# ArtOfBBQ/debigulator

Measured on NVIDIA B200. Metric: inflate_output_GBps, higher is better.
Workload: dtype u8

## Files before the change

debigulator_b200/csrc/bsplit_kernels.cuh:

```cuda
#pragma once
#include <cuda_runtime.h>
#include <stdint.h>

#include "bsplit_core.h"
#include "split_kernels.cuh"

namespace dbg {

constexpr uint64_t BS_MIN_BYTES = 65536;
constexpr int BS_WARPS_PER_CTA = 4;

struct BsSummary {
    uint32_t n_split;
    uint32_t total_regions;
    uint64_t total_in;
    uint64_t cells_used;
    uint32_t n_fallback;
    uint32_t pad;
    uint64_t split_in;
    uint64_t tok_bytes;
    uint32_t n_pruned;
    uint32_t pad2;
};

// ... 62 lines not shown
    if (thr < b.min_bytes) thr = b.min_bytes;
    if (b.dyn_all && size >= b.min_bytes && ((b.pre_status && b.pre_status[s]) ? 0u : ((b.in_base[b.in_off[s]] >> 1) & 3)) == 2) thr = b.min_bytes;
    uint32_t flag = 0;
    const bool ok = (!b.pre_status || b.pre_status[s] == 0) && (!b.taken || b.taken[s] == 0) && size >= thr && cap >= size &&
                    size < (1ull << 31) && cap < (1ull << 32) - 1024;
    b.redo[s] = 0;
    const uint32_t first = ok ? b.in_base[b.in_off[s]] : 0u;
    if (ok && ((first >> 1) & 3) != 0 && (first & 1) == 0) {
        flag = 1;
        atomicAdd(&b.summary->n_split, 1u);
        atomicAdd((unsigned long long *)&b.summary->split_in, (unsigned long long)size);
    }
    b.flag[s] = flag;
}

__global__ void bs_assign_kernel(BsBatch b)
{
    const uint32_t s = blockIdx.x * blockDim.x + threadIdx.x;
    if (s >= b.n || !b.flag[s]) return;
    const uint32_t nreg = (uint32_t)((b.in_size[s] + b.region_bytes - 1) / b.region_bytes);
    b.chunk_base[s] = atomicAdd(&b.summary->total_regions, nreg);
    b.nchunks[s] = nreg;
    if (b.tok)
        b.tok_stream_base[s] = (uint64_t)b.tok_per_byte *
                               atomicAdd((unsigned long long *)&b.summary->tok_bytes, (unsigned long long)b.in_size[s]);
}

__global__ void bs_fill_kernel(BsBatch b)
{
    const uint32_t s = blockIdx.x;
    if (!b.flag[s]) return;
    const uint32_t nch = b.nchunks[s], base = b.chunk_base[s];
    for (uint32_t c = threadIdx.x; c < nch; c += blockDim.x) b.chunk_stream[base + c] = s;
}

__global__ void __launch_bounds__(BS_WARPS_PER_CTA * 32) bs_search_kernel(BsBatch b)
{
    const uint32_t total_regions = b.summary->total_regions;
    __shared__ uint16_t kraft12[4096];
    __shared__ SearchSmem qs[BS_WARPS_PER_CTA];
    build_kraft12(kraft12, threadIdx.x, blockDim.x);
    __syncthreads();
    SearchSmem *q = &qs[threadIdx.x >> 5];
    const uint32_t warps = gridDim.x * BS_WARPS_PER_CTA;
    for (uint32_t t = blockIdx.x * BS_WARPS_PER_CTA + (threadIdx.x >> 5); t < total_regions; t += warps) {
        const uint32_t s = b.chunk_stream[t], c = t - b.chunk_base[s];
        uint64_t cand = 0;
        if (c) cand = find_block_start(q, kraft12, b.in_base + b.in_off[s], b.in_size[s], (uint64_t)c * b.region_bytes * 8,
                                       (uint64_t)(c + 1) * b.region_bytes * 8);
        if (simt::lane() == 0) b.cand[t] = cand;
        simt::syncwarp();
    }
}

__global__ void bs_prune_kernel(BsBatch b)
{
    const uint32_t s = blockIdx.x * blockDim.x + threadIdx.x;
    if (s >= b.n || !b.flag[s]) return;
    const uint32_t nch = b.nchunks[s], base = b.chunk_base[s];
    const uint64_t bits = 8 * b.in_size[s];
    uint64_t prev = 0, worst = 0;
    for (uint32_t c = 1; c < nch; c++) {
        const uint64_t cand = b.cand[base + c];
        if (cand == BS_NONE) continue;
        if (cand - prev > worst) worst = cand - prev;
        prev = cand;
    }
    if (bits - prev > worst) worst = bits - prev;
    if (worst > bits / 3) {
        for (uint32_t c = 0; c < nch; c++) b.cand[base + c] = BS_NONE;
        b.redo[s] = 1;
        atomicAdd(&b.summary->n_pruned, 1u);
    }
}

__device__ __forceinline__ uint64_t bs_next_hint(const BsBatch &b, uint32_t s, uint32_t t)
{
    const uint32_t end = b.chunk_base[s] + b.nchunks[s];
    for (uint32_t u = t + 1; u < end; u++)
        if (b.cand[u] != BS_NONE) return b.cand[u];
    return BS_NONE;
}

__global__ void __launch_bounds__(BS_WARPS_PER_CTA * 32) bs_count_kernel(BsBatch b)
{
    const uint32_t total_regions = b.summary->total_regions;
    extern __shared__ __align__(16) uint8_t smem_raw[];
    InflateSmem *sm = reinterpret_cast<InflateSmem *>(smem_raw) + (threadIdx.x >> 5);
    const uint32_t warps = gridDim.x * BS_WARPS_PER_CTA;
    for (uint32_t t = blockIdx.x * BS_WARPS_PER_CTA + (threadIdx.x >> 5); t < total_regions; t += warps) {
        const uint64_t start = b.cand[t];
        if (start == BS_NONE) continue;
        const uint32_t s = b.chunk_stream[t];
        const uint64_t next = bs_next_hint(b, s, t);
        ChunkResult r;
        if (b.tok)
            r = decode_block_chunk<SINK_TOKENS>(sm, b.in_base + b.in_off[s], b.in_size[s], start, next, nullptr, 0, 0,
                                                b.tok + bs_tok_base(b, s, start), bs_tok_cap(b, s, start, next), b.lanes != 0,
                                                b.lb_stats);
        else
            r = decode_block_chunk<SINK_COUNT>(sm, b.in_base + b.in_off[s], b.in_size[s], start, next, nullptr, 0, 0);
        if (simt::lane() == 0) {
            b.exit_bits[t] = r.exit_bits;
            b.c_out_len[t] = r.out_bytes;
            b.c_flag[t] = r.flag;
            if (b.tok) b.c_ntok[t] = r.ntok;
        }
        simt::syncwarp();
    }
}

__global__ void bs_chain_kernel(BsBatch b)
{
    const uint32_t s = blockIdx.x * blockDim.x + threadIdx.x;
    if (s >= b.n || !b.flag[s] || b.redo[s]) return;
    const uint32_t nch = b.nchunks[s], base = b.chunk_base[s];
    const uint64_t cap = b.out_cap[s];
    uint64_t pos = 0, expected = 0;
    uint32_t st = ST_OK;
    bool ended = false, fail = false;
    for (uint32_t c = 0; c < nch; c++) {
        const uint32_t t = base + c;
        const uint64_t cand = b.cand[t];
        const uint32_t len = b.c_out_len[t], flag = b.c_flag[t];
        b.c_out_off[t] = pos;
        if (cand == BS_NONE || ended || fail) {
            b.c_flag[t] = CH_IDLE;
            b.c_out_len[t] = 0;
            continue;
        }
        if (cand < expected) {
            b.c_flag[t] = CH_IDLE;
            b.c_out_len[t] = 0;
            continue;
        }
        if (cand != expected) {
            fail = true;
            b.c_flag[t] = CH_IDLE;
            b.c_out_len[t] = 0;
            continue;
        }
        if (flag >= CH_ERR) {
            st = pos + len > cap ? (uint32_t)ST_OUT_OVERFLOW : flag - CH_ERR;
            ended = true;
            b.c_flag[t] = CH_IDLE;
            b.c_out_len[t] = 0;
            continue;
        }
        pos += len;
        if (pos > cap) {
            st = ST_OUT_OVERFLOW;
            ended = true;
        } else if (flag != CH_RUN) {
            ended = true;
        } else {
            expected = b.exit_bits[t];
        }
    }
    if (!ended) fail = true;
    if (fail) {
        for (uint32_t c = 0; c < nch; c++) {
            b.c_flag[base + c] = CH_IDLE;
            b.c_out_len[base + c] = 0;
        }
        b.redo[s] = 1;
        b.cell_base[s] = 0;
        atomicAdd(&b.summary->n_fallback, 1u);
// ... 134 lines not shown
```

debigulator_b200/csrc/dbg_api.cu:

```cuda
#include <cuda_runtime.h>
#include <stdarg.h>
#include <stdint.h>
#include <stdio.h>
#include <stdlib.h>
#include <string.h>

#include <algorithm>
#include <atomic>
#include <condition_variable>
#include <deque>
#include <mutex>
#include <numeric>
#include <thread>
#include <utility>
#include <vector>

#include "../../include/debigulator_b200.h"
#include "bmp_kernels.cuh"
#include "bsplit_kernels.cuh"
#include "fx_kernels.cuh"
#include "kernels.cuh"
#include "png_kernels.cuh"
#include "split_kernels.cuh"
#include "sprite_kernels.cuh"
// ... 192 lines not shown
    if (const char *v = getenv("DBG_FX_CHUNK")) ctx->fx_chunk_forced = (uint32_t)std::min(1 << 20, std::max((int)dbg::FX_MIN_CHUNK, atoi(v))) & ~15u;
    if (const char *v = getenv("DBG_FX_GROUP")) ctx->fx_group_forced = (uint32_t)std::min(1 << 22, std::max(4096, atoi(v))) & ~15u;
    if (const char *v = getenv("DBG_FX")) ctx->fx = atoi(v) != 0;
    if (const char *v = getenv("DBG_FX_EXPAND_CTAS")) ctx->fx_expand_ctas = (uint32_t)std::min(16, std::max(1, atoi(v)));
    if (const char *v = getenv("DBG_WAVES")) ctx->waves = std::min((int)dbg_ctx::MAX_WAVES, std::max(1, atoi(v)));
    if (const char *v = getenv("DBG_PNG_WAVES")) ctx->png_waves = std::min((int)dbg_ctx::MAX_WAVES, std::max(1, atoi(v)));
    if (const char *v = getenv("DBG_BSPLIT")) ctx->bsplit = atoi(v) != 0;
    if (const char *v = getenv("DBG_BSPLIT_LANES")) ctx->bsplit_lanes = atoi(v) != 0;
    if (const char *v = getenv("DBG_BS_PIECES")) ctx->bs_pieces = atoi(v) != 0;
    if (const char *v = getenv("DBG_ROUNDS")) ctx->rounds = atoi(v) != 0;
    if (const char *v = getenv("DBG_ROUND_BITS")) ctx->round_bits = (uint32_t)std::min(1 << 20, std::max(8192, atoi(v)));
    if (const char *v = getenv("DBG_BSPLIT_ALL")) ctx->bsplit_all = atoi(v);
    if (const char *v = getenv("DBG_BSPLIT_FACTOR_Q")) ctx->bsplit_factor_q = (uint32_t)std::max(1, atoi(v));
    if (const char *v = getenv("DBG_BSPLIT_TOKENS")) ctx->bsplit_tok_per_byte = (uint32_t)std::min(8, std::max(0, atoi(v)));
    if (const char *v = getenv("DBG_BSPLIT_REGION")) ctx->bsplit_region = (uint32_t)std::min(1 << 20, std::max(4096, atoi(v)));
    if (const char *v = getenv("DBG_BSPLIT_REGION_MIN")) ctx->bsplit_region_min = (uint32_t)std::min((int)ctx->bsplit_region, std::max(4096, atoi(v)));
    if (const char *v = getenv("DBG_BSPLIT_MIN_BYTES")) ctx->bsplit_min_bytes = std::max<uint64_t>(strtoull(v, nullptr, 10), 2 * (uint64_t)ctx->bsplit_region);
    if (const char *v = getenv("DBG_INFLATE_CTAS_PER_SM")) {
        int k = atoi(v);
        if (k >= 1 && k <= dbg::INFLATE_CTAS_PER_SM) ctx->inflate_ctas_per_sm = (uint32_t)k;
    }
    return ctx;
}

extern "C" dbg_ctx *dbg_create(int device) { return ctx_create(device, nullptr, 0, nullptr); }

extern "C" void dbg_destroy(dbg_ctx *ctx)
{
    if (!ctx) return;
    cudaSetDevice(ctx->device);
    cudaDeviceSynchronize();
    Buf *all[] = {&ctx->d_in, &ctx->d_out, &ctx->d_desc, &ctx->h_in, &ctx->h_out, &ctx->h_desc, &ctx->d_stats};
    for (Buf *b : all) b->release();
    for (int i = 0; i < dbg_ctx::MAX_WAVES; i++) {
        ctx->slot[i].release();
        Slot &sl = ctx->slot[i];
        if (sl.stream) cudaStreamDestroy(sl.stream);
        if (sl.done) cudaEventDestroy(sl.done);
        if (sl.uploaded) cudaEventDestroy(sl.uploaded);
        if (sl.aux_stream) cudaStreamDestroy(sl.aux_stream);
        if (sl.aux_fork) cudaEventDestroy(sl.aux_fork);
        if (sl.aux_join) cudaEventDestroy(sl.aux_join);
    }
    for (auto &pe : ctx->prof_events) {
        cudaEventDestroy(pe.first);
        cudaEventDestroy(pe.second);
    }
    if (ctx->wave_ready) cudaEventDestroy(ctx->wave_ready);
    if (ctx->up_stream) cudaStreamDestroy(ctx->up_stream);
    if (ctx->stream) cudaStreamDestroy(ctx->stream);
    delete ctx;
}

extern "C" int dbg_bsplit_stats(const dbg_ctx *ctx, uint64_t *streams, uint64_t *fallbacks)
{
    if (!ctx) return DBG_ERR_NO_DEVICE;
    if (streams) *streams = ctx->bs_streams;
    if (fallbacks) *fallbacks = ctx->bs_fallbacks;
    return DBG_OK;
}

extern "C" int dbg_fx_stats(const dbg_ctx *ctx, uint64_t *streams, uint64_t *handed_back, uint64_t *extra_runs)
{
    if (!ctx) return DBG_ERR_NO_DEVICE;
    uint64_t v[3] = {0, 0, 0};
    if (cudaSetDevice(ctx->device) != cudaSuccess || cudaDeviceSynchronize() != cudaSuccess ||
        cudaMemcpy(v, ctx->d_stats.p, sizeof(v), cudaMemcpyDeviceToHost) != cudaSuccess)
        return DBG_ERR_CUDA;
    if (streams) *streams = v[0];
    if (handed_back) *handed_back = v[1];
    if (extra_runs) *extra_runs = v[2];
    return DBG_OK;
}

extern "C" int dbg_lane_stats(const dbg_ctx *ctx, uint32_t v[8])
{
    if (!ctx || !v) return DBG_ERR_ARG;
    if (cudaSetDevice(ctx->device) != cudaSuccess || cudaDeviceSynchronize() != cudaSuccess ||
        cudaMemcpy(v, (uint64_t *)ctx->d_stats.p + 4, 5 * sizeof(uint32_t), cudaMemcpyDeviceToHost) != cudaSuccess ||
        cudaMemcpy(v + 5, (uint64_t *)ctx->d_stats.p + 8, 3 * sizeof(uint32_t), cudaMemcpyDeviceToHost) != cudaSuccess)
        return DBG_ERR_CUDA;
    return DBG_OK;
}

extern "C" int dbg_set_verify(dbg_ctx *ctx, int on)
{
    if (!ctx) return DBG_ERR_ARG;
    ctx->verify = on != 0;
    return DBG_OK;
}

extern "C" int dbg_trim(dbg_ctx *ctx)
{
    if (!ctx) return DBG_ERR_ARG;
    CU(cudaSetDevice(ctx->device));
    CU(cudaDeviceSynchronize());
    for (int i = 0; i < dbg_ctx::MAX_WAVES; i++) ctx->slot[i].release();
    Buf *all[] = {&ctx->d_in, &ctx->d_out, &ctx->d_desc, &ctx->h_in, &ctx->h_out, &ctx->h_desc};
    for (Buf *b : all) b->release();
    return DBG_OK;
}

extern "C" int dbg_profile_enable(dbg_ctx *ctx, int on)
{
    if (!ctx) return DBG_ERR_ARG;
    ctx->profiling = on != 0;
    ctx->prof_used = 0;
    return DBG_OK;
}

extern "C" int dbg_profile_read_tag(dbg_ctx *ctx, int tag, double *total_ms, uint64_t *launches)
{
    if (!ctx || !total_ms || !launches) return DBG_ERR_ARG;
    CU(cudaSetDevice(ctx->device));
    double sum = 0;
    uint64_t cnt = 0;
    for (size_t i = 0; i < ctx->prof_used; i++) {
        if (ctx->prof_tag[i] != tag) continue;
        float ms = 0;
        CU(cudaEventSynchronize(ctx->prof_events[i].second));
        CU(cudaEventElapsedTime(&ms, ctx->prof_events[i].first, ctx->prof_events[i].second));
        sum += ms;
        cnt++;
    }
    *total_ms = sum;
    *launches = cnt;
    return DBG_OK;
}

extern "C" int dbg_profile_read(dbg_ctx *ctx, double *total_ms, uint64_t *launches)
{
    int rc = dbg_profile_read_tag(ctx, DBG_PROF_INFLATE, total_ms, launches);
    if (rc == DBG_OK) ctx->prof_used = 0;
    return rc;
}

extern "C" int dbg_synchronize(dbg_ctx *ctx)
{
    if (!ctx) return DBG_ERR_ARG;
    CU(cudaSetDevice(ctx->device));
    CU(cudaStreamSynchronize(ctx->stream));
    return DBG_OK;
}

struct ProfScope {
    dbg_ctx *ctx;
    cudaStream_t s;
    cudaEvent_t e1 = nullptr;
    ProfScope(dbg_ctx *c, cudaStream_t st, int tag) : ctx(c), s(st)
    {
        if (!ctx->profiling) return;
        std::lock_guard<std::mutex> lock(ctx->prof_mu);
        if (ctx->prof_used == ctx->prof_events.size()) {
            cudaEvent_t a = nullptr, b = nullptr;
            if (cudaEventCreate(&a) != cudaSuccess || cudaEventCreate(&b) != cudaSuccess) return;
            ctx->prof_events.push_back({a, b});
            ctx->prof_tag.push_back(0);
        }
        ctx->prof_tag[ctx->prof_used] = tag;
        cudaEventRecord(ctx->prof_events[ctx->prof_used].first, s);
        e1 = ctx->prof_events[ctx->prof_used].second;
        ctx->prof_used++;
    }
    ~ProfScope()
    {
        if (e1) cudaEventRecord(e1, s);
// ... 1489 lines not shown
```

debigulator_b200/csrc/inflate_core.h:

```cpp
#pragma once
#include "simt.h"

namespace dbg {

enum InflateStatus : uint32_t {
    ST_OK = 0,
    ST_CAP_LT_INPUT = 1,
    ST_INPUT_TOO_SMALL = 2,
    ST_TOO_LARGE = 3,
    ST_STORED_LEN = 4,
    ST_BAD_TABLE = 5,
    ST_BAD_CODE = 6,
    ST_BAD_SYMBOL = 7,
    ST_BAD_DISTANCE = 8,
    ST_OUT_OVERFLOW = 9,
    ST_TRUNCATED = 10,
    ST_BAD_REPEAT = 11,
    ST_CONTAINER = 12,
};

struct InflateSmem {
    uint32_t ring[256];
    uint32_t lit_lut[512];
    uint32_t dist_lut[256];
    uint16_t lit_sorted[288];
    uint16_t lit_first[16], lit_offs[16], lit_cnt[16];
    uint16_t dist_first[16], dist_offs[16], dist_cnt[16];
    uint8_t dist_sorted[32];
    uint8_t lens[320];
    uint32_t cand[2][64];
};

enum { E_LIT = 0x10, E_EOB = 0x20, E_BASE = 0x40, E_BAD = 0x80 };
enum { K_CLEN = 0, K_LITLEN = 1, K_DIST = 2 };
enum { LIT_ROOT = 9, DIST_ROOT = 8 };

template <int KIND>
DBG_DEV uint32_t make_entry(uint32_t sym, uint32_t l)
{
    if (KIND == K_CLEN) return (sym << 16) | E_LIT | l;
    if (KIND == K_LITLEN) {
        if (sym < 256) return (sym << 16) | E_LIT | l;
        if (sym == 256) return E_EOB | l;
        if (sym > 285) return E_BAD | l;
        uint32_t i = sym - 257, xb, base;
        if (i < 8) { xb = 0; base = 3 + i; }
        else if (i == 28) { xb = 0; base = 258; }
        else { xb = (i >> 2) - 1; base = 3 + ((4 + (i & 3)) << xb); }
        return (base << 16) | (xb << 8) | E_BASE | l;
    }
    if (sym > 29) return E_BAD | l;
    uint32_t xb = sym < 4 ? 0 : (sym >> 1) - 1;
    uint32_t base = sym < 4 ? sym + 1 : 1 + ((2 + (sym & 1)) << xb);
    return (base << 16) | (xb << 8) | E_BASE | l;
}

struct Window {
    const uint8_t *base;
    uint32_t *ring;
    uint32_t end16;
    uint32_t w0, w1, w2, w3;
    uint32_t wb;
    uint32_t s;
    int32_t wleft;
    uint32_t lim_w, lim_b;

    DBG_DEVM void load_chunk(uint32_t c)
    {
        uint32_t off = (c << 9) + ((uint32_t)simt::lane() << 4);
        bool in = off < end16;
        simt::cp_async16_stream(&ring[((c & 1) << 7) + ((uint32_t)simt::lane() << 2)], base + (in ? off : 0), in ? 16 : 0);
    }
    DBG_DEVM void maintain()
    {
        if (wb & 64) {
            simt::cp_async_wait_all();
            simt::syncwarp();
        } else {
            simt::syncwarp();
            load_chunk((wb >> 7) + 1);
            simt::cp_async_commit();
        }
    }
    DBG_DEVM void shift()
    {
        w0 = w1;
        w1 = w2;
        w2 = w3;
        wb++;
        wleft--;
        if ((wb & 63) == 0) maintain();
        w3 = ring[(wb + 3) & 255];
    }
    DBG_DEVM uint32_t peek32() const { return simt::funnel_r(w0, w1, s); }
    DBG_DEVM void consume(uint32_t n)
    {
        s += n;
        while (s >= 32) {
            s -= 32;
            shift();
        }
    }
    DBG_DEVM uint64_t abs_bits() const { return ((uint64_t)wb << 5) + s; }
    DBG_DEVM void seek(uint64_t bytepos)
    {
        uint32_t c = (uint32_t)(bytepos >> 9);
        simt::cp_async_wait_all();
        simt::syncwarp();
        load_chunk(c);
        load_chunk(c + 1);
        simt::cp_async_commit();
        simt::cp_async_wait_all();
        simt::syncwarp();
// ... 369 lines not shown
        simt::syncwarp();
    } else {
        uint32_t v = w.peek32();
        hlit = (v & 31) + 257;
        hdist = ((v >> 5) & 31) + 1;
        uint32_t hclen = ((v >> 10) & 15) + 4;
        w.consume(14);
        if (ln < 19) sm->lens[ln] = 0;
        simt::syncwarp();
        for (uint32_t i = 0; i < hclen; i++) {
            if (ln == 0) sm->lens[swizzle_at(i)] = (uint8_t)(w.peek32() & 7);
            w.consume(3);
        }
        simt::syncwarp();
        uint32_t cl_max;
        if (!build_table<K_CLEN, uint8_t>(sm->lens, 19, 7, sm->dist_lut, sm->dist_sorted, sm->dist_first, sm->dist_offs,
                                          sm->dist_cnt, &cl_max))
            return ST_BAD_TABLE;
        const uint32_t n = hlit + hdist;
        uint32_t i = 0, prev = 0;
        while (i < n) {
            uint32_t bits = w.peek32();
            uint32_t e = sm->dist_lut[bits & 127];
            uint32_t l = e & 15;
            if (l == 0) return ST_BAD_CODE;
            uint32_t sym = e >> 16;
            if (sym < 16) {
                w.consume(l);
                if (ln == 0) sm->lens[i] = (uint8_t)sym;
                prev = sym;
                i++;
                continue;
            }
            uint32_t rep, val;
            if (sym == 16) {
                if (i == 0) return ST_BAD_REPEAT;
                rep = 3 + ((bits >> l) & 3);
                w.consume(l + 2);
                val = prev;
            } else if (sym == 17) {
                rep = 3 + ((bits >> l) & 7);
                w.consume(l + 3);
                val = 0;
            } else {
                rep = 11 + ((bits >> l) & 127);
                w.consume(l + 7);
                val = 0;
            }
            for (uint32_t k = ln; k < rep; k += 32)
                if (i + k < n) sm->lens[i + k] = (uint8_t)val;
            prev = val;
            i += rep;
        }
        simt::syncwarp();
    }
    if (!build_table<K_LITLEN, uint16_t>(sm->lens, (int)hlit, LIT_ROOT, sm->lit_lut, sm->lit_sorted, sm->lit_first,
                                         sm->lit_offs, sm->lit_cnt, &bt.lit_max))
        return ST_BAD_TABLE;
    if (!build_table<K_DIST, uint8_t>(sm->lens + hlit, (int)hdist, DIST_ROOT, sm->dist_lut, sm->dist_sorted, sm->dist_first,
                                      sm->dist_offs, sm->dist_cnt, &bt.dist_max))
        return ST_BAD_TABLE;
    return ST_OK;
}

template <int SINK>
DBG_DEV uint32_t decode_symbols(Window &w, InflateSmem *sm, const BlockTables &bt, Sink &k, uint32_t &end_reason)
{
    const uint32_t ln = (uint32_t)simt::lane();
    uint32_t flip = 0;
    simt::syncwarp();
    for (;;) {
        const bool two = w.wleft >= 2;
        uint32_t lim = two ? 64u : 32u;
        if (w.wleft <= 0) {
            lim = w.wleft == 0 ? w.lim_b : 0u;
            if (w.s >= lim) {
                end_reason = END_LIMIT;
                return ST_OK;
            }
        }
        const uint32_t lo = simt::funnel_r(w.w0, w.w1, ln);
        const uint32_t mid = simt::funnel_r(w.w1, w.w2, ln);
        const uint32_t hi = simt::funnel_r(w.w2, w.w3, ln);
        uint32_t *cand = sm->cand[flip];
        flip ^= 1;
        cand[ln] = decode_candidate(sm, lo, mid, ln);
        if (two) cand[ln + 32] = decode_candidate(sm, mid, hi, ln + 32);
        simt::syncwarp();
        uint32_t p = w.s, cur, err = 0;
        bool eob = false, slow = false;
        const bool roomy = SINK == SINK_COUNT || SINK == SINK_TOKENS || k.cap - k.pos >= 64 * 258;
#define DBG_SYM(CHECK)                                                                         \
            cur = p;                                                                           \
            {                                                                                  \
                const uint32_t info = cand[p];                                                 \
                const uint32_t lf = (info >> 7) & 511;                                         \
                p = info & 127;                                                                \
                if (lf == 0) {                                                                 \
                    err = emit_literal<SINK, CHECK>(k, info >> 16);                            \
                    if (CHECK && err) break;                                                   \
                } else if (lf >= 3) {                                                          \
                    err = emit_match<SINK, CHECK>(k, lf, (info >> 16) + 1);                    \
                    if (err) break;                                                            \
                } else {                                                                       \
                    const uint32_t code = info >> 16;                                          \
                    if (code == CAND_EOB) eob = true;                                          \
                    else if (code == CAND_ERR) err = ST_BAD_SYMBOL;                            \
                    else slow = true;  \
                    break;                                                                     \
                }                                                                              \
            }
#define DBG_WALK(CHECK)                                                                        \
        do {                                                                                   \
            DBG_SYM(CHECK)                                                                     \
            if (p >= lim) break;                                                               \
            DBG_SYM(CHECK)                                                                     \
            if (p >= lim) break;                                                               \
            DBG_SYM(CHECK)                                                                     \
            if (p >= lim) break;                                                               \
            DBG_SYM(CHECK)                                                                     \
        } while (p < lim)
        if (roomy) DBG_WALK(false);
        else DBG_WALK(true);
#undef DBG_WALK
#undef DBG_SYM
        if (err) return err;
        if (slow) {
            if (cur >= 32) {
                w.shift();
                cur -= 32;
            }
            w.s = cur;
            uint32_t bits = w.peek32();
            uint32_t e = sm->lit_lut[bits & ((1u << LIT_ROOT) - 1)];
            if ((e & 15) == 0) {
                e = slow_decode<K_LITLEN, uint16_t>(bits, LIT_ROOT, bt.lit_max, sm->lit_sorted, sm->lit_first, sm->lit_offs,
                                                    sm->lit_cnt);
                if (!e) return ST_BAD_CODE;
            }
            w.consume(e & 15);
            if (e & E_LIT) {
                err = emit_literal<SINK, true>(k, e >> 16);
                if (err) return err;
                continue;
            }
            if (e & E_EOB) {
                end_reason = END_EOB;
                return ST_OK;
            }
            if (e & E_BAD) return ST_BAD_SYMBOL;
            bits = w.peek32();
            uint32_t xb = (e >> 8) & 31;
            uint32_t len = (e >> 16) + (bits & ((1u << xb) - 1));
            w.consume(xb);
            bits = w.peek32();
            e = sm->dist_lut[bits & ((1u << DIST_ROOT) - 1)];
            if ((e & 15) == 0) {
                e = slow_decode<K_DIST, uint8_t>(bits, DIST_ROOT, bt.dist_max, sm->dist_sorted, sm->dist_first, sm->dist_offs,
                                                 sm->dist_cnt);
                if (!e) return ST_BAD_CODE;
            }
            if (e & E_BAD) return ST_BAD_SYMBOL;
            xb = (e >> 8) & 31;
            uint32_t l2 = e & 15;
            uint32_t dist = (e >> 16) + ((bits >> l2) & ((1u << xb) - 1));
            w.consume(l2 + xb);
            err = emit_match<SINK, true>(k, len, dist);
            if (err) return err;
            continue;
        }
        w.s = p & 31;
        for (uint32_t n = p >> 5; n; n--) w.shift();
        if (eob) {
            end_reason = END_EOB;
            return ST_OK;
        }
        if (!two && lim < 32) {
            end_reason = END_LIMIT;
            return ST_OK;
        }
    }
}

struct StreamIn {
    uint32_t mis;
    uint64_t end_byte;
    uint64_t q2_limit;
};

DBG_DEV StreamIn open_stream(Window &w, InflateSmem *sm, const uint8_t *in, uint64_t in_size)
{
    StreamIn g;
    g.mis = (uint32_t)((uintptr_t)in & 15);
    g.end_byte = (uint64_t)g.mis + in_size;
    g.q2_limit = 8 * g.end_byte - 7;
    w.base = in - g.mis;
    w.ring = sm->ring;
    w.end16 = (uint32_t)((g.end_byte + 15) & ~15ull);
    w.lim_w = (uint32_t)(g.q2_limit >> 5);
    w.lim_b = (uint32_t)g.q2_limit & 31;
    return g;
}

DBG_DEV void copy_stored_u16(uint16_t *dst, const uint8_t *src, uint32_t len)
{
    for (uint32_t i = (uint32_t)simt::lane(); i < len; i += 32) dst[i] = src[i];
}

struct LaneBits {
    const uint32_t *a;
    uint32_t boff;
    uint32_t last;
    uint32_t widx;
    uint32_t nxt;
    uint32_t nb;
    uint64_t buf;

    DBG_DEVM uint32_t word(uint32_t i) const { return i <= last ? simt::ldg_u32(a + i) : 0u; }
    DBG_DEVM void open(const uint8_t *in, uint64_t in_size)
    {
        const uintptr_t p = (uintptr_t)in;
        a = (const uint32_t *)(p & ~(uintptr_t)3);
        boff = 8 * (uint32_t)(p & 3);
        last = (uint32_t)((((p + in_size + 15) & ~(uintptr_t)15) - (p & ~(uintptr_t)3)) >> 2) - 1;
    }
    DBG_DEVM void seek(uint64_t stream_bit)
    {
        const uint64_t abit = stream_bit + boff;
        widx = (uint32_t)(abit >> 5);
        const uint32_t sh = (uint32_t)abit & 31;
        const uint64_t two = (uint64_t)word(widx) | ((uint64_t)word(widx + 1) << 32);
        buf = two >> sh;
        nb = 64 - sh;
        widx += 2;
        nxt = word(widx);
    }
    DBG_DEVM void refill()
    {
        if (nb <= 32) {
            buf |= (uint64_t)nxt << nb;
            widx++;
            nb += 32;
            nxt = word(widx);
        }
    }
    DBG_DEVM void drop(uint32_t n)
    {
        buf >>= n;
        nb -= n;
    }
};

struct TokOut {
    uint32_t *p;
    uint32_t q0, q1, q2;
    uint32_t k;
    DBG_DEVM void open(uint32_t *dst)
    {
        p = dst;
        q0 = q1 = q2 = 0;
        k = 0;
    }
    DBG_DEVM void put(uint32_t t)
    {
        if (k == 3) {
            simt::st_u32x4(p, q0, q1, q2, t);
            p += 4;
            k = 0;
        } else if (k == 0 && ((uintptr_t)p & 15)) {
            *p++ = t;
        } else {
            q0 = q1;
            q1 = q2;
            q2 = t;
            k++;
        }
    }
    DBG_DEVM void close()
    {
        if (k == 3) *p++ = q0;
        if (k >= 2) *p++ = q1;
        if (k >= 1) *p++ = q2;
        k = 0;
    }
};

enum : uint32_t { CH_RUN = 0, CH_EOB = 1, CH_Q2 = 2, CH_IDLE = 3, CH_ERR = 16 };

constexpr uint32_t LB_MIN_SUB = 2048;
constexpr uint32_t LB_MAX_EXTENT = 1u << 20;
constexpr uint32_t LB_TOKENS_STRETCH = 4096;
constexpr uint32_t LB_NOHINT_EXTENT = 3u << 17;
constexpr uint32_t LB_ROUND_BITS = 86016;
constexpr uint32_t LB_ROUND_TOKENS = 16384;
constexpr uint32_t LB_MERGE_BITS = 1024;
constexpr uint32_t LB_STARTS = 48;
enum : uint32_t { LBK_LIT = 0, LBK_MATCH = 1, LBK_EOB = 2, LBK_BAD = 3 };

DBG_DEV uint32_t lb_symbol(const InflateSmem *sm, const BlockTables &bt, LaneBits &br, uint32_t *nbits, uint32_t *len, uint32_t *tok)
{
    br.refill();
    uint32_t x = (uint32_t)br.buf;
    uint32_t e = sm->lit_lut[x & ((1u << LIT_ROOT) - 1)];
    if ((e & 15) == 0) {
        e = slow_decode<K_LITLEN, uint16_t>(x, LIT_ROOT, bt.lit_max, sm->lit_sorted, sm->lit_first, sm->lit_offs, sm->lit_cnt);
        if (!e) return LBK_BAD;
    }
    const uint32_t l1 = e & 15;
    *len = 1;
    *tok = e >> 16;
    *nbits = l1;
    if (e & E_LIT) {
        br.drop(l1);
        return LBK_LIT;
    }
    if (e & E_EOB) {
        br.drop(l1);
        return LBK_EOB;
    }
    if (!(e & E_BASE)) return LBK_BAD;
    const uint32_t xb = (e >> 8) & 31;
    const uint32_t ln = (e >> 16) + ((x >> l1) & ((1u << xb) - 1));
    br.drop(l1 + xb);
    br.refill();
    x = (uint32_t)br.buf;
    uint32_t e2 = sm->dist_lut[x & ((1u << DIST_ROOT) - 1)];
    if ((e2 & 15) == 0) {
        e2 = slow_decode<K_DIST, uint8_t>(x, DIST_ROOT, bt.dist_max, sm->dist_sorted, sm->dist_first, sm->dist_offs, sm->dist_cnt);
        if (!e2) return LBK_BAD;
    }
    if (!(e2 & E_BASE)) return LBK_BAD;
    const uint32_t l2 = e2 & 15, xb2 = (e2 >> 8) & 31;
    const uint32_t dist = (e2 >> 16) + ((x >> l2) & ((1u << xb2) - 1));
    br.drop(l2 + xb2);
    *nbits = l1 + xb + l2 + xb2;
    *len = ln;
    *tok = TOKEN_MATCH | (ln << 16) | (dist - 1);
    return LBK_MATCH;
}

DBG_DEV uint64_t lb_merge_point(const InflateSmem *sm, const BlockTables &bt, const uint8_t *base16, uint64_t end_byte, uint64_t s0,
                                uint32_t give_up, uint64_t q2_limit)
{
    LaneBits br;
    br.open(base16, end_byte);
    br.seek(s0);
    uint64_t reach = (1ull << LB_STARTS) - 1;
    uint64_t anchor = s0;
    for (uint32_t steps = 0; steps < 2 * LB_STARTS + give_up / 2; steps++) {
        if (reach == 0) return ~0ull;
        const uint32_t lo32 = (uint32_t)reach;
        const uint32_t p = lo32 ? (uint32_t)simt::ffs(lo32) - 1 : 31 + (uint32_t)simt::ffs((uint32_t)(reach >> 32));
        if ((reach >> p) == 1) return anchor + p;
        if (p) {
            uint32_t r = p;
            if (r > 32) {
                br.refill();
                br.drop(32);
                r -= 32;
            }
            br.refill();
            br.drop(r);
            anchor += p;
            reach >>= p;
        }
        if (anchor - s0 > give_up) return ~0ull;
        reach &= ~1ull;
        if (anchor >= q2_limit) continue;
        LaneBits t = br;
        uint32_t nbits, len, tok;
        const uint32_t kind = lb_symbol(sm, bt, t, &nbits, &len, &tok);
        if (kind == LBK_LIT || kind == LBK_MATCH) reach |= 1ull << nbits;
    }
    return ~0ull;
}

enum : uint32_t { LB_UNUSED = 0, LB_DONE = 1, LB_PARTIAL = 2 };
#ifdef DBG_SIMT_EMU
static uint32_t g_lb_done = 0, g_lb_tried = 0, g_lb_partial = 0;
#endif

struct LaneRound {
    uint32_t ntok;
    uint32_t out;
    uint64_t resume;
    uint32_t used;
    uint32_t stride;
    uint32_t mine;
};

template <bool COMPACT>
DBG_DEV uint32_t lane_round(const InflateSmem *sm, const BlockTables &bt, const uint8_t *base16, const StreamIn &g, uint64_t p0, uint64_t ext,
                            uint32_t *area, uint32_t area_cap, LaneRound &r, uint32_t *stats)
{
    const uint32_t ln = (uint32_t)simt::lane();
    r.ntok = 0;
    r.out = 0;
    r.resume = p0;
    r.used = 0;
    r.stride = 0;
    r.mine = 0;
    if (ext > LB_MAX_EXTENT) ext = LB_MAX_EXTENT;
    if (ext < 4 * LB_MIN_SUB) return LB_UNUSED;
    uint32_t sub = ((uint32_t)ext + 31) / 32;
    if (sub < LB_MIN_SUB) sub = LB_MIN_SUB;
    sub = (sub + 31) & ~31u;
    const uint32_t L = ((uint32_t)ext + sub - 1) / sub;
    const uint32_t stride = area_cap / L;
    if (stride < sub / 16) return LB_UNUSED;
#ifdef DBG_SIMT_EMU
    if (ln == 0) g_lb_tried++;
#else
    if (ln == 0 && stats) atomicAdd(&stats[0], 1u);
#endif
    uint64_t entry = p0;
    const uint32_t give_up = sub / 2 < LB_MERGE_BITS ? sub / 2 : LB_MERGE_BITS;
    if (ln > 0 && ln < L) entry = lb_merge_point(sm, bt, base16, g.end_byte, p0 + (uint64_t)ln * sub, give_up, g.q2_limit);
    if (ln >= L) entry = ~0ull;
    const uint32_t e_lo = simt::shfl_down((uint32_t)entry, 1), e_hi = simt::shfl_down((uint32_t)(entry >> 32), 1);
    uint64_t target = ((uint64_t)e_hi << 32) | e_lo;
    const bool has_target = ln + 1 < L && target != ~0ull;
    if (!has_target) target = p0 + (uint64_t)(ln + 1) * sub;
    enum : uint32_t { R_ARRIVED = 0, R_EOB = 1, R_STOPPED = 2, R_BROKEN = 3 };
    uint32_t n = 0, out = 0, flag = R_BROKEN;
    uint64_t pos = entry;
    if (entry != ~0ull) {
        LaneBits br;
        br.open(base16, g.end_byte);
        br.seek(entry);
        TokOut wr;
        wr.open(area + (uint64_t)ln * stride);
        flag = R_ARRIVED;
        while (pos < target) {
            if (pos >= g.q2_limit || n >= stride) {
                flag = R_BROKEN;
                break;
            }
            uint32_t nbits, len, tok;
            const uint32_t kind = lb_symbol(sm, bt, br, &nbits, &len, &tok);
            if (kind == LBK_BAD) {
                flag = R_BROKEN;
                break;
            }
            pos += nbits;
            if (kind == LBK_EOB) {
                flag = R_EOB;
                break;
            }
            wr.put(tok);
            n++;
            out += len;
        }
        wr.close();
        if (flag == R_ARRIVED) {
            if (!has_target) flag = R_STOPPED;
            else if (pos != target) flag = R_BROKEN;
        }
    }
    const uint32_t stops = simt::ballot(flag != R_ARRIVED);
    const uint32_t stop_lane = (uint32_t)simt::ffs(stops) - 1;
    const uint32_t stop_flag = simt::shfl(flag, (int)stop_lane);
    const uint32_t used = stop_flag == R_BROKEN ? stop_lane : stop_lane + 1;
    if (used == 0) return LB_UNUSED;
    r.used = used;
    r.stride = stride;
    uint32_t in = ln < used ? n : 0u, io = ln < used ? out : 0u;
    const uint32_t mine = in;
    r.mine = mine;
    for (int d = 1; d < 32; d <<= 1) {
        const uint32_t yn = simt::shfl_up(in, d), yo = simt::shfl_up(io, d);
        if (ln >= (uint32_t)d) {
            in += yn;
            io += yo;
        }
    }
    r.ntok = simt::shfl(in, 31);
    r.out = simt::shfl(io, 31);
    const uint64_t res = stop_flag == R_BROKEN ? entry : pos;
    r.resume = ((uint64_t)simt::shfl((uint32_t)(res >> 32), (int)stop_lane) << 32) | simt::shfl((uint32_t)res, (int)stop_lane);
    simt::syncwarp();
    for (uint32_t j = 1; COMPACT && j < used; j++) {
        const uint32_t cnt = simt::shfl(mine, (int)j), dst0 = simt::shfl(in - mine, (int)j);
        const uint32_t *src = area + (uint64_t)j * stride;
        for (uint32_t i0 = 0; i0 < cnt; i0 += 128) {
            uint32_t v[4];
#pragma unroll
            for (int k = 0; k < 4; k++) {
                const uint32_t i = i0 + 32 * k + ln;
                v[k] = i < cnt ? src[i] : 0u;
            }
            simt::syncwarp();
#pragma unroll
            for (int k = 0; k < 4; k++) {
                const uint32_t i = i0 + 32 * k + ln;
                if (i < cnt) area[dst0 + i] = v[k];
            }
            simt::syncwarp();
        }
    }
    const bool whole = stop_flag == R_EOB;
#ifdef DBG_SIMT_EMU
    if (ln == 0) (whole ? g_lb_done : g_lb_partial)++;
#else
    if (ln == 0 && stats) atomicAdd(&stats[whole ? 1 : 2], 1u);
#endif
    return whole ? LB_DONE : LB_PARTIAL;
}

DBG_DEV uint32_t expand_tokens_bytes(const uint32_t *tok, uint32_t ntok, uint8_t *out, uint32_t &pos_io, uint32_t cap)
{
    const uint32_t ln = (uint32_t)simt::lane();
    uint32_t pos = pos_io;
    uint32_t t_next = ln < ntok ? tok[ln] : 0u;
    for (uint32_t base = 0; base < ntok; base += 32) {
        const bool have = base + ln < ntok;
        const uint32_t t = t_next;
        t_next = base + 32 + ln < ntok ? tok[base + 32 + ln] : 0u;
        const bool is_match = have && (t & TOKEN_MATCH);
        const uint32_t len = !have ? 0u : is_match ? (t >> 16) & 0x1ff : 1u;
        const uint32_t dist = (t & 0x7fff) + 1;
        uint32_t incl = len;
        for (int d = 1; d < 32; d <<= 1) {
            const uint32_t y = simt::shfl_up(incl, d);
            if (ln >= (uint32_t)d) incl += y;
        }
        const uint32_t o = pos + incl - len;
        const uint32_t total = simt::shfl(incl, 31);
        const bool bad_dist = is_match && dist > o;
        const bool over = have && (uint64_t)o + len > cap;
        const uint32_t fails = simt::ballot(bad_dist || over);
        if (fails) {
            const int f = simt::ffs(fails) - 1;
            pos_io = pos;
            return simt::shfl(over ? (uint32_t)ST_OUT_OVERFLOW : (uint32_t)ST_BAD_DISTANCE, f);
        }
        simt::syncwarp();
        if (have && !is_match) out[o] = (uint8_t)t;
        const bool free_m = is_match && len <= 16 && o + len <= pos + dist;
        if (free_m) {
            const uint8_t *src = out + (o - dist);
            uint8_t *dst = out + o;
            uint32_t v[16];
#pragma unroll
            for (int j = 0; j < 16; j++) v[j] = (uint32_t)j < len ? src[j] : 0u;
#pragma unroll
            for (int j = 0; j < 16; j++)
                if ((uint32_t)j < len) dst[j] = (uint8_t)v[j];
        }
        uint32_t m = simt::ballot(is_match && !free_m);
        while (m) {
            const int j = simt::ffs(m) - 1;
            m &= m - 1;
            copy_match_slow(out, simt::shfl(o, j), simt::shfl(len, j), simt::shfl(dist, j));
        }
        pos += total;
    }
    simt::syncwarp();
    pos_io = pos;
    return ST_OK;
}

enum { BLK_FINAL = 0, BLK_Q2 = 1, BLK_STOP = 2 };
template <int SINK>
DBG_DEV uint32_t inflate_blocks(Window &w, const StreamIn &g, InflateSmem *sm, Sink &k, uint64_t stop_bit, uint32_t &end)
{
    BlockTables bt;
    bt.lit_max = bt.dist_max = 0;
    end = BLK_FINAL;
    for (;;) {
        if (w.abs_bits() >= stop_bit) {
            end = BLK_STOP;
            return ST_OK;
        }
        if (w.abs_bits() >= 8 * g.end_byte) return ST_TRUNCATED;
        const uint32_t hdr = w.peek32() & 7;
        w.consume(3);
        const bool more = !(hdr & 1);
        const uint32_t btype = hdr >> 1;
        if (btype == 0) {
            w.consume((0u - w.s) & 7);
            const uint32_t v = w.peek32();
            const uint32_t len = v & 0xffff, nlen = v >> 16;
            w.consume(32);
            if (len != (~nlen & 0xffff)) return ST_STORED_LEN;
            if (len) {
                const uint64_t bytepos = w.abs_bits() >> 3;
                if (bytepos + len > g.end_byte) return ST_TRUNCATED;
                if (SINK == SINK_TOKENS) {
                    if (len > 256) {
                        k.tok_cap = 0;
                        k.ntok = 0x40000000u;
                    } else {
                        const uint8_t *src = w.base + bytepos;
                        for (uint32_t i = (uint32_t)simt::lane(); i < len; i += 32)
                            if (k.ntok + i < k.tok_cap) k.tok[k.ntok + i] = src[i];
                        k.ntok += len;
                    }
                } else if (SINK != SINK_COUNT) {
                    if ((uint64_t)k.pos + len > k.cap) return ST_OUT_OVERFLOW;
                    if (SINK == SINK_BYTES) {
                        copy_stored(k.out + k.pos, w.base + bytepos, len);
                    } else {
                        flush_pending16(k.pd);
                        copy_stored_u16(k.out16 + k.pos, w.base + bytepos, len);
                        simt::syncwarp();
                    }
                }
                k.pos += len;
                w.seek(bytepos + len);
            }
        } else if (btype != 3) {
            uint32_t st = read_huffman_tables(w, sm, btype, bt);
            if (st) return st;
            uint32_t why = END_EOB;
            bool block_done = false;
            bool use_lanes = (SINK == SINK_TOKENS || SINK == SINK_BYTES) && k.lanes;
            if (use_lanes && k.lane_skip) {
                k.lane_skip--;
                use_lanes = false;
            }
            for (;;) {
                bool stretch = false;
                if (use_lanes) {
                    for (;;) {
                        const uint64_t p0 = w.abs_bits();
                        const uint64_t in_end = 8 * g.end_byte;
                        LaneRound lr;
                        uint32_t got;
                        if (SINK == SINK_TOKENS) {
                            const bool hinted = stop_bit < in_end;
                            uint64_t ext = (hinted ? stop_bit : in_end) > p0 ? (hinted ? stop_bit : in_end) - p0 : 0;
                            if (!hinted && ext > LB_NOHINT_EXTENT) ext = LB_NOHINT_EXTENT;
                            if (k.ntok >= k.tok_cap) {
                                use_lanes = false;
                                break;
                            }
                            got = lane_round<true>(sm, bt, w.base, g, p0, ext, k.tok + k.ntok, k.tok_cap - k.ntok, lr, k.lb_stats);
                            if (got == LB_UNUSED) {
                                use_lanes = false;
                                break;
                            }
                            k.ntok += lr.ntok;
                            k.pos += lr.out;
                        } else {
                            uint64_t ext = in_end > p0 ? in_end - p0 : 0;
                            if (ext > k.round_bits) ext = k.round_bits;
                            got = lane_round<false>(sm, bt, w.base, g, p0, ext, k.tok, k.tok_cap, lr, k.lb_stats);
                            if (got == LB_UNUSED) {
                                if (ext >= 4 * LB_MIN_SUB) {
                                    k.lane_skip = k.lane_bad < 8 ? k.lane_bad : 8;
                                    k.lane_bad++;
                                    stretch = true;
                                } else {
                                    use_lanes = false;
                                }
                                break;
                            }
                            simt::syncwarp();
                            flush_pending(k.pd);
                            for (uint32_t j = 0; j < lr.used; j++) {
                                st = expand_tokens_bytes(k.tok + (uint64_t)j * lr.stride, simt::shfl(lr.mine, (int)j), k.out, k.pos, k.cap);
                                if (st) return st;
                            }
                        }
                        w.seek_bits(lr.resume);
                        if (got == LB_DONE) {
                            block_done = true;
                            k.lane_bad = 0;
                            break;
                        }
                        if (SINK == SINK_TOKENS) {
                            if (lr.used > 2) stretch = true;
                            else use_lanes = false;
                            break;
                        }
                        if (lr.resume - p0 < k.round_bits / 2) {
                            if (lr.used <= 2) {
                                k.lane_skip = k.lane_bad < 8 ? k.lane_bad : 8;
                                k.lane_bad++;
                            }
                            stretch = true;
                            break;
                        }
                        k.lane_bad = 0;
                    }
                    if (block_done) break;
                    if (k.lane_skip) use_lanes = false;
                }
                bool temp_limit = false;
                if ((SINK == SINK_BYTES || SINK == SINK_TOKENS) && use_lanes && stretch) {
                    const uint64_t lim = w.abs_bits() + (SINK == SINK_BYTES ? k.round_bits / 4 : LB_TOKENS_STRETCH);
                    if (lim < g.q2_limit) {
                        w.set_limit(lim);
                        temp_limit = true;
                    }
                }
                why = END_EOB;
                st = decode_symbols<SINK>(w, sm, bt, k, why);

                if (temp_limit) w.set_limit(g.q2_limit);
                if (st) return st;
                if (temp_limit && why == END_LIMIT) continue;
                break;
            }
            if (block_done) {
                if (!more) return ST_OK;
                continue;
            }
            if (why == END_LIMIT) {
                end = BLK_Q2;
                return ST_OK;
            }
        }
        if (!more) return ST_OK;
    }
}

DBG_DEV uint32_t inflate_warp(InflateSmem *sm, const uint8_t *in, uint64_t in_size, uint8_t *out, uint64_t cap,
                              uint64_t *final_size, uint32_t *tok_scratch = nullptr, uint32_t *lb_stats = nullptr,
                              uint32_t round_bits = LB_ROUND_BITS)
{
    *final_size = 0;
    if (cap < in_size) return ST_CAP_LT_INPUT;
    if (in_size < 5) return ST_INPUT_TOO_SMALL;
    if (in_size >= (1ull << 31) || cap >= (1ull << 32) - 1024) return ST_TOO_LARGE;

    Window w;
    const StreamIn g = open_stream(w, sm, in, in_size);
    w.seek(g.mis);

    Sink k;
    k.out = out;
    k.out16 = nullptr;
    k.abs_base = 0;
    k.pos = 0;
    k.cap = (uint32_t)cap;
    k.pd.ptr = out;
    k.pd.val = 0;
    k.pd.on = false;
    k.tok = tok_scratch;
    k.ntok = 0;
    k.tok_cap = tok_scratch ? LB_ROUND_TOKENS : 0;
    k.lanes = tok_scratch != nullptr;
    k.lb_stats = lb_stats;
    k.round_bits = round_bits;
    k.lane_bad = k.lane_skip = 0;
    uint32_t end;
    const uint32_t st = inflate_blocks<SINK_BYTES>(w, g, sm, k, ~0ull, end);
    if (st) return st;
    flush_pending(k.pd);
    *final_size = k.pos;
    return ST_OK;
}

struct ChunkResult {
    uint64_t exit_bits;
    uint32_t out_bytes;
    uint32_t flag;
    uint32_t ntok;
};

DBG_DEV bool is_single_fixed_block(const uint8_t *in) { return (in[0] & 7) == 3; }


}
```

Before: 129.5.

## Replace per-lane merge-point search with shared sync bitmaps in lane rounds

Lane-parallel decoding previously found each sub-range's entry point by running a 48-way reachability merge search before decoding. Now each lane decodes from its start, recording every visited bit position in a shared-memory bitmap (unioned with the walk ring/cand buffers to save space). It then runs forward until it hits a position the next lane also visited, and token counts before that sync point are skipped via popcount. This removes the redundant merge-point pass, at the cost of extra shared writes, a slightly different resume/partial policy, and a minBlocks=5 launch bound on the count kernel. Optional phase-clock instrumentation is also added behind a macro.

```diff
diff --git a/debigulator_b200/csrc/bsplit_kernels.cuh b/debigulator_b200/csrc/bsplit_kernels.cuh
--- a/debigulator_b200/csrc/bsplit_kernels.cuh
+++ b/debigulator_b200/csrc/bsplit_kernels.cuh
@@ -168,7 +168,7 @@
     return BS_NONE;
 }
 
-__global__ void __launch_bounds__(BS_WARPS_PER_CTA * 32) bs_count_kernel(BsBatch b)
+__global__ void __launch_bounds__(BS_WARPS_PER_CTA * 32, 5) bs_count_kernel(BsBatch b)
 {
     const uint32_t total_regions = b.summary->total_regions;
     extern __shared__ __align__(16) uint8_t smem_raw[];
diff --git a/debigulator_b200/csrc/dbg_api.cu b/debigulator_b200/csrc/dbg_api.cu
--- a/debigulator_b200/csrc/dbg_api.cu
+++ b/debigulator_b200/csrc/dbg_api.cu
@@ -298,6 +298,20 @@
         return DBG_ERR_CUDA;
     return DBG_OK;
 }
+
+#ifdef DBG_PHASE_CLOCKS
+extern "C" int dbg_phase_clocks(uint64_t v[dbg::PH_N], int reset)
+{
+    if (!v) return DBG_ERR_ARG;
+    if (cudaDeviceSynchronize() != cudaSuccess || cudaMemcpyFromSymbol(v, dbg::g_phase_clk, sizeof(uint64_t) * dbg::PH_N) != cudaSuccess)
+        return DBG_ERR_CUDA;
+    if (reset) {
+        const uint64_t zero[dbg::PH_N] = {};
+        if (cudaMemcpyToSymbol(dbg::g_phase_clk, zero, sizeof(zero)) != cudaSuccess) return DBG_ERR_CUDA;
+    }
+    return DBG_OK;
+}
+#endif
 
 extern "C" int dbg_set_verify(dbg_ctx *ctx, int on)
 {
diff --git a/debigulator_b200/csrc/inflate_core.h b/debigulator_b200/csrc/inflate_core.h
--- a/debigulator_b200/csrc/inflate_core.h
+++ b/debigulator_b200/csrc/inflate_core.h
@@ -19,8 +19,17 @@
     ST_CONTAINER = 12,
 };
 
+constexpr uint32_t LB_SYNC_WORDS = 29;
+constexpr uint32_t LB_SYNC_BITS = LB_SYNC_WORDS * 32;
+
 struct InflateSmem {
-    uint32_t ring[256];
+    union {
+        struct {
+            uint32_t ring[256];
+            uint32_t cand[2][64];
+        } walk;
+        uint32_t sync_bm[32][LB_SYNC_WORDS];
+    };
     uint32_t lit_lut[512];
     uint32_t dist_lut[256];
     uint16_t lit_sorted[288];
@@ -28,7 +37,6 @@
     uint16_t dist_first[16], dist_offs[16], dist_cnt[16];
     uint8_t dist_sorted[32];
     uint8_t lens[320];
-    uint32_t cand[2][64];
 };
 
 enum { E_LIT = 0x10, E_EOB = 0x20, E_BASE = 0x40, E_BAD = 0x80 };
@@ -564,7 +572,7 @@
         const uint32_t lo = simt::funnel_r(w.w0, w.w1, ln);
         const uint32_t mid = simt::funnel_r(w.w1, w.w2, ln);
         const uint32_t hi = simt::funnel_r(w.w2, w.w3, ln);
-        uint32_t *cand = sm->cand[flip];
+        uint32_t *cand = sm->walk.cand[flip];
         flip ^= 1;
         cand[ln] = decode_candidate(sm, lo, mid, ln);
         if (two) cand[ln + 32] = decode_candidate(sm, mid, hi, ln + 32);
@@ -677,7 +685,7 @@
     g.end_byte = (uint64_t)g.mis + in_size;
     g.q2_limit = 8 * g.end_byte - 7;
     w.base = in - g.mis;
-    w.ring = sm->ring;
+    w.ring = sm->walk.ring;
     w.end16 = (uint32_t)((g.end_byte + 15) & ~15ull);
     w.lim_w = (uint32_t)(g.q2_limit >> 5);
     w.lim_b = (uint32_t)g.q2_limit & 31;
@@ -767,6 +775,19 @@
     }
 };
 
+enum { PH_TABLES = 0, PH_ENTRY = 1, PH_RUNS = 2, PH_EXPAND = 3, PH_WALK = 4, PH_STORED = 5, PH_TOTAL = 6, PH_N = 8 };
+#if defined(DBG_PHASE_CLOCKS) && !defined(DBG_SIMT_EMU)
+__device__ unsigned long long g_phase_clk[PH_N];
+#define DBG_PHASE_T0(t) const long long t = clock64()
+#define DBG_PHASE_ADD(cond, i, t)                                                                         \
+    do {                                                                                                  \
+        if ((cond) && simt::lane() == 0) atomicAdd(&g_phase_clk[i], (unsigned long long)(clock64() - (t))); \
+    } while (0)
+#else
+#define DBG_PHASE_T0(t)
+#define DBG_PHASE_ADD(cond, i, t) do {} while (0)
+#endif
+
 enum : uint32_t { CH_RUN = 0, CH_EOB = 1, CH_Q2 = 2, CH_IDLE = 3, CH_ERR = 16 };
 
 constexpr uint32_t LB_MIN_SUB = 2048;
@@ -775,8 +796,6 @@
 constexpr uint32_t LB_NOHINT_EXTENT = 3u << 17;
 constexpr uint32_t LB_ROUND_BITS = 86016;
 constexpr uint32_t LB_ROUND_TOKENS = 16384;
-constexpr uint32_t LB_MERGE_BITS = 1024;
-constexpr uint32_t LB_STARTS = 48;
 enum : uint32_t { LBK_LIT = 0, LBK_MATCH = 1, LBK_EOB = 2, LBK_BAD = 3 };
 
 DBG_DEV uint32_t lb_symbol(const InflateSmem *sm, const BlockTables &bt, LaneBits &br, uint32_t *nbits, uint32_t *len, uint32_t *tok)
@@ -821,45 +840,10 @@
     return LBK_MATCH;
 }
 
-DBG_DEV uint64_t lb_merge_point(const InflateSmem *sm, const BlockTables &bt, const uint8_t *base16, uint64_t end_byte, uint64_t s0,
-                                uint32_t give_up, uint64_t q2_limit)
-{
-    LaneBits br;
-    br.open(base16, end_byte);
-    br.seek(s0);
-    uint64_t reach = (1ull << LB_STARTS) - 1;
-    uint64_t anchor = s0;
-    for (uint32_t steps = 0; steps < 2 * LB_STARTS + give_up / 2; steps++) {
-        if (reach == 0) return ~0ull;
-        const uint32_t lo32 = (uint32_t)reach;
-        const uint32_t p = lo32 ? (uint32_t)simt::ffs(lo32) - 1 : 31 + (uint32_t)simt::ffs((uint32_t)(reach >> 32));
-        if ((reach >> p) == 1) return anchor + p;
-        if (p) {
-            uint32_t r = p;
-            if (r > 32) {
-                br.refill();
-                br.drop(32);
-                r -= 32;
-            }
-            br.refill();
-            br.drop(r);
-            anchor += p;
-            reach >>= p;
-        }
-        if (anchor - s0 > give_up) return ~0ull;
-        reach &= ~1ull;
-        if (anchor >= q2_limit) continue;
-        LaneBits t = br;
-        uint32_t nbits, len, tok;
-        const uint32_t kind = lb_symbol(sm, bt, t, &nbits, &len, &tok);
-        if (kind == LBK_LIT || kind == LBK_MATCH) reach |= 1ull << nbits;
-    }
-    return ~0ull;
-}
-
 enum : uint32_t { LB_UNUSED = 0, LB_DONE = 1, LB_PARTIAL = 2 };
 #ifdef DBG_SIMT_EMU
 static uint32_t g_lb_done = 0, g_lb_tried = 0, g_lb_partial = 0;
+static uint64_t g_lr_stats[8];
 #endif
 
 struct LaneRound {
@@ -867,12 +851,12 @@
     uint32_t out;
     uint64_t resume;
     uint32_t used;
-    uint32_t stride;
+    uint32_t start;
     uint32_t mine;
 };
 
 template <bool COMPACT>
-DBG_DEV uint32_t lane_round(const InflateSmem *sm, const BlockTables &bt, const uint8_t *base16, const StreamIn &g, uint64_t p0, uint64_t ext,
+DBG_DEV uint32_t lane_round(InflateSmem *sm, const BlockTables &bt, const uint8_t *base16, const StreamIn &g, uint64_t p0, uint64_t ext,
                             uint32_t *area, uint32_t area_cap, LaneRound &r, uint32_t *stats)
 {
     const uint32_t ln = (uint32_t)simt::lane();
@@ -880,7 +864,7 @@
     r.out = 0;
     r.resume = p0;
     r.used = 0;
-    r.stride = 0;
+    r.start = 0;
     r.mine = 0;
     if (ext > LB_MAX_EXTENT) ext = LB_MAX_EXTENT;
     if (ext < 4 * LB_MIN_SUB) return LB_UNUSED;
@@ -890,64 +874,134 @@
     const uint32_t L = ((uint32_t)ext + sub - 1) / sub;
     const uint32_t stride = area_cap / L;
     if (stride < sub / 16) return LB_UNUSED;
+    simt::cp_async_wait_all();
+    simt::syncwarp();
 #ifdef DBG_SIMT_EMU
     if (ln == 0) g_lb_tried++;
+    uint32_t iters = 0;
 #else
     if (ln == 0 && stats) atomicAdd(&stats[0], 1u);
 #endif
-    uint64_t entry = p0;
-    const uint32_t give_up = sub / 2 < LB_MERGE_BITS ? sub / 2 : LB_MERGE_BITS;
-    if (ln > 0 && ln < L) entry = lb_merge_point(sm, bt, base16, g.end_byte, p0 + (uint64_t)ln * sub, give_up, g.q2_limit);
-    if (ln >= L) entry = ~0ull;
-    const uint32_t e_lo = simt::shfl_down((uint32_t)entry, 1), e_hi = simt::shfl_down((uint32_t)(entry >> 32), 1);
-    uint64_t target = ((uint64_t)e_hi << 32) | e_lo;
-    const bool has_target = ln + 1 < L && target != ~0ull;
-    if (!has_target) target = p0 + (uint64_t)(ln + 1) * sub;
+    DBG_PHASE_T0(t_entry);
     enum : uint32_t { R_ARRIVED = 0, R_EOB = 1, R_STOPPED = 2, R_BROKEN = 3 };
-    uint32_t n = 0, out = 0, flag = R_BROKEN;
-    uint64_t pos = entry;
-    if (entry != ~0ull) {
-        LaneBits br;
-        br.open(base16, g.end_byte);
-        br.seek(entry);
-        TokOut wr;
-        wr.open(area + (uint64_t)ln * stride);
-        flag = R_ARRIVED;
-        while (pos < target) {
-            if (pos >= g.q2_limit || n >= stride) {
-                flag = R_BROKEN;
+    const uint32_t s0 = ln * sub;
+    const uint32_t q2 = g.q2_limit - p0 < 0xffffffffull ? (uint32_t)(g.q2_limit - p0) : 0xffffffffu;
+    for (uint32_t i = 0; i < LB_SYNC_WORDS; i++) sm->sync_bm[ln][i] = 0;
+    uint32_t n = 0, out = 0, flag = ln < L ? R_ARRIVED : R_BROKEN;
+    uint32_t rp = s0;
+    LaneBits br;
+    br.open(base16, g.end_byte);
+    TokOut wr;
+    wr.open(area + (uint64_t)ln * stride);
+    if (flag == R_ARRIVED) br.seek(p0 + rp);
+    while (flag == R_ARRIVED && rp < s0 + LB_SYNC_BITS) {
+        if (rp >= q2 || n >= stride) {
+            flag = R_BROKEN;
+            break;
+        }
+        if (ln > 0) sm->sync_bm[ln][(rp - s0) >> 5] |= 1u << ((rp - s0) & 31);
+        uint32_t nbits, len, tok;
+        const uint32_t kind = lb_symbol(sm, bt, br, &nbits, &len, &tok);
+#ifdef DBG_SIMT_EMU
+        iters++;
+#endif
+        if (kind == LBK_BAD || kind == LBK_EOB) {
+            if (ln == 0) {
+                flag = kind == LBK_EOB ? R_EOB : R_BROKEN;
+                rp += nbits;
                 break;
             }
-            uint32_t nbits, len, tok;
-            const uint32_t kind = lb_symbol(sm, bt, br, &nbits, &len, &tok);
-            if (kind == LBK_BAD) {
-                flag = R_BROKEN;
+            for (uint32_t i = 0; i <= (rp - s0) >> 5; i++) sm->sync_bm[ln][i] = 0;
+            n = out = 0;
+            wr.open(area + (uint64_t)ln * stride);
+            rp += 1;
+            if (rp >= s0 + LB_SYNC_BITS) flag = R_BROKEN;
+            else br.seek(p0 + rp);
+            continue;
+        }
+        rp += nbits;
+        wr.put(tok);
+        n++;
+        out += len;
+    }
+    simt::syncwarp();
+    DBG_PHASE_ADD(!COMPACT, PH_ENTRY, t_entry);
+    DBG_PHASE_T0(t_runs);
+    while (flag == R_ARRIVED) {
+        if (rp >= s0 + sub) {
+            const uint32_t off = rp - (s0 + sub);
+            if (ln + 1 >= L || off >= LB_SYNC_BITS) {
+                flag = R_STOPPED;
                 break;
             }
-            pos += nbits;
-            if (kind == LBK_EOB) {
-                flag = R_EOB;
-                break;
-            }
-            wr.put(tok);
-            n++;
-            out += len;
-        }
-        wr.close();
-        if (flag == R_ARRIVED) {
-            if (!has_target) flag = R_STOPPED;
-            else if (pos != target) flag = R_BROKEN;
-        }
-    }
+            if ((sm->sync_bm[ln + 1][off >> 5] >> (off & 31)) & 1) break;
+        }
+        if (rp >= q2 || n >= stride) {
+            flag = R_BROKEN;
+            break;
+        }
+        uint32_t nbits, len, tok;
+        const uint32_t kind = lb_symbol(sm, bt, br, &nbits, &len, &tok);
+#ifdef DBG_SIMT_EMU
+        iters++;
+#endif
+        if (kind == LBK_BAD) {
+            flag = R_BROKEN;
+            break;
+        }
+        rp += nbits;
+        if (kind == LBK_EOB) {
+            flag = R_EOB;
+            break;
+        }
+        wr.put(tok);
+        n++;
+        out += len;
+    }
+    wr.close();
     const uint32_t stops = simt::ballot(flag != R_ARRIVED);
     const uint32_t stop_lane = (uint32_t)simt::ffs(stops) - 1;
     const uint32_t stop_flag = simt::shfl(flag, (int)stop_lane);
     const uint32_t used = stop_flag == R_BROKEN ? stop_lane : stop_lane + 1;
-    if (used == 0) return LB_UNUSED;
+    const uint32_t prev = simt::shfl_up(rp, 1);
+    const uint32_t entry = ln == 0 ? 0u : prev;
+    uint32_t first = 0;
+    if (ln > 0 && ln <= stop_lane) {
+        const uint32_t off = entry - s0;
+        for (uint32_t i = 0; i < (off >> 5); i++) first += (uint32_t)simt::popc(sm->sync_bm[ln][i]);
+        first += (uint32_t)simt::popc(sm->sync_bm[ln][off >> 5] & ((1u << (off & 31)) - 1));
+        if (COMPACT && ln < used) {
+            const uint32_t *t = area + (uint64_t)ln * stride;
+            for (uint32_t i = 0; i < first; i++) out -= (t[i] & TOKEN_MATCH) ? (t[i] >> 16) & 0x1ff : 1u;
+        }
+    }
+    DBG_PHASE_ADD(!COMPACT, PH_RUNS, t_runs);
+#ifdef DBG_SIMT_EMU
+    if (!COMPACT) {
+        uint32_t mi = iters, ms = ln < stop_lane ? rp - (s0 + sub) : 0u, all = iters;
+        const uint32_t lost = simt::popc(simt::ballot(flag == R_STOPPED && ln + 1 < L));
+        for (int d = 16; d; d >>= 1) {
+            const uint32_t a = simt::shfl_xor(mi, d), b = simt::shfl_xor(ms, d);
+            mi = a > mi ? a : mi;
+            ms = b > ms ? b : ms;
+            all += simt::shfl_xor(all, d);
+        }
+        if (ln == 0) {
+            g_lr_stats[0]++;
+            g_lr_stats[1] += mi;
+            if (mi > g_lr_stats[2]) g_lr_stats[2] = mi;
+            g_lr_stats[3] += ms;
+            if (ms > g_lr_stats[4]) g_lr_stats[4] = ms;
+            g_lr_stats[5] += all;
+            g_lr_stats[7] += lost;
+        }
+    }
+#endif
+    if (used == 0) return LB_PARTIAL;
     r.used = used;
-    r.stride = stride;
-    uint32_t in = ln < used ? n : 0u, io = ln < used ? out : 0u;
+    uint32_t in = ln < used ? n - first : 0u, io = ln < used ? out : 0u;
     const uint32_t mine = in;
+    r.start = ln * stride + first;
     r.mine = mine;
     for (int d = 1; d < 32; d <<= 1) {
         const uint32_t yn = simt::shfl_up(in, d), yo = simt::shfl_up(io, d);
@@ -958,12 +1012,11 @@
     }
     r.ntok = simt::shfl(in, 31);
     r.out = simt::shfl(io, 31);
-    const uint64_t res = stop_flag == R_BROKEN ? entry : pos;
-    r.resume = ((uint64_t)simt::shfl((uint32_t)(res >> 32), (int)stop_lane) << 32) | simt::shfl((uint32_t)res, (int)stop_lane);
+    r.resume = p0 + simt::shfl(stop_flag == R_BROKEN ? entry : rp, (int)stop_lane);
     simt::syncwarp();
     for (uint32_t j = 1; COMPACT && j < used; j++) {
         const uint32_t cnt = simt::shfl(mine, (int)j), dst0 = simt::shfl(in - mine, (int)j);
-        const uint32_t *src = area + (uint64_t)j * stride;
+        const uint32_t *src = area + (uint64_t)j * stride + simt::shfl(first, (int)j);
         for (uint32_t i0 = 0; i0 < cnt; i0 += 128) {
             uint32_t v[4];
 #pragma unroll
@@ -1068,6 +1121,7 @@
             if (len) {
                 const uint64_t bytepos = w.abs_bits() >> 3;
                 if (bytepos + len > g.end_byte) return ST_TRUNCATED;
+                DBG_PHASE_T0(t_stored);
                 if (SINK == SINK_TOKENS) {
                     if (len > 256) {
                         k.tok_cap = 0;
@@ -1090,10 +1144,13 @@
                 }
                 k.pos += len;
                 w.seek(bytepos + len);
+                DBG_PHASE_ADD(SINK == SINK_BYTES, PH_STORED, t_stored);
             }
         } else if (btype != 3) {
+            DBG_PHASE_T0(t_tables);
             uint32_t st = read_huffman_tables(w, sm, btype, bt);
             if (st) return st;
+            DBG_PHASE_ADD(SINK == SINK_BYTES, PH_TABLES, t_tables);
             uint32_t why = END_EOB;
             bool block_done = false;
             bool use_lanes = (SINK == SINK_TOKENS || SINK == SINK_BYTES) && k.lanes;
@@ -1138,12 +1195,14 @@
                                 }
                                 break;
                             }
+                            DBG_PHASE_T0(t_expand);
                             simt::syncwarp();
                             flush_pending(k.pd);
                             for (uint32_t j = 0; j < lr.used; j++) {
-                                st = expand_tokens_bytes(k.tok + (uint64_t)j * lr.stride, simt::shfl(lr.mine, (int)j), k.out, k.pos, k.cap);
+                                st = expand_tokens_bytes(k.tok + simt::shfl(lr.start, (int)j), simt::shfl(lr.mine, (int)j), k.out, k.pos, k.cap);
                                 if (st) return st;
                             }
+                            DBG_PHASE_ADD(true, PH_EXPAND, t_expand);
                         }
                         w.seek_bits(lr.resume);
                         if (got == LB_DONE) {
@@ -1178,10 +1237,15 @@
                     }
                 }
                 why = END_EOB;
+                DBG_PHASE_T0(t_walk);
                 st = decode_symbols<SINK>(w, sm, bt, k, why);
+                DBG_PHASE_ADD(SINK == SINK_BYTES, PH_WALK, t_walk);
 
                 if (temp_limit) w.set_limit(g.q2_limit);
                 if (st) return st;
+#ifdef DBG_SIMT_EMU
+                if (SINK == SINK_BYTES && temp_limit && simt::lane() == 0) g_lr_stats[6]++;
+#endif
                 if (temp_limit && why == END_LIMIT) continue;
                 break;
             }
@@ -1228,7 +1292,9 @@
     k.round_bits = round_bits;
     k.lane_bad = k.lane_skip = 0;
     uint32_t end;
+    DBG_PHASE_T0(t_total);
     const uint32_t st = inflate_blocks<SINK_BYTES>(w, g, sm, k, ~0ull, end);
+    DBG_PHASE_ADD(true, PH_TOTAL, t_total);
     if (st) return st;
     flush_pending(k.pd);
     *final_size = k.pos;
```

Result: faster. 136.9, median of 6 (+5.7%).
